# dmMaze/comic-text-detector

Measured on NVIDIA H100. Metric: pages/sec @1024x1024 synthetic, higher is better.
Workload: dtype fp16

## Files before the change

### comic-text-detector_b200/binding.py

```python
import ctypes as C
import os

import numpy as np

_HERE = os.path.dirname(os.path.abspath(__file__))
LIB_PATH = os.path.join(_HERE, "libctd_b200.so")
MAX_SRC = 3
ABI_VERSION = 2
PREC_FP16_TC, PREC_FP32_SIMT, PREC_FP16_SIMT, PREC_SPLIT_TC = 0, 1, 2, 3


class CtdOp(C.Structure):
    _fields_ = [("kind", C.c_int32), ("n_src", C.c_int32), ("src_buf", C.c_int32 * MAX_SRC),
                ("src_coff", C.c_int32 * MAX_SRC), ("src_c", C.c_int32 * MAX_SRC), ("dst_buf", C.c_int32),
                ("dst_coff", C.c_int32), ("cout", C.c_int32), ("cout_pad", C.c_int32), ("ksize", C.c_int32),
                ("stride", C.c_int32), ("act", C.c_int32), ("residual", C.c_int32), ("aux", C.c_int32),
                ("w16_off", C.c_int64), ("w32_off", C.c_int64), ("b_off", C.c_int64), ("p_off", C.c_int64)]


class CtdBufDesc(C.Structure):
    _fields_ = [("channels", C.c_int32), ("down", C.c_int32)]


class CtdConfig(C.Structure):
# ... 38 lines not shown
class CtdDevicePage(C.Structure):
    _fields_ = [("data", C.c_void_p), ("stride_h", C.c_int64), ("stride_w", C.c_int64), ("stride_c", C.c_int64),
                ("event", C.c_void_p)]


EXPORTS = ["ctd_create", "ctd_destroy", "ctd_last_error", "ctd_forward", "ctd_get_net_outputs", "ctd_get_mask_u8",
           "ctd_get_detections", "ctd_get_db_components", "ctd_last_forward_ms", "ctd_last_launch_count",
           "ctd_debug_read_buffer", "ctd_debug_write_buffer", "ctd_connected_components", "ctd_nms",
           "ctd_timer_start", "ctd_timer_stop", "ctd_profile_forward", "ctd_get_device_outputs",
           "ctd_get_text_lines", "ctd_seg_represent", "ctd_refine_mask", "ctd_submit", "ctd_collect",
           "ctd_results_bytes", "ctd_join", "ctd_forward_resized", "ctd_get_mask_u8_resized",
           "ctd_resize_linear_u8", "ctd_debug_run_ops", "ctd_get_nms_status", "ctd_group_output",
           "ctd_expand_textwindow", "ctd_detect_page", "ctd_results_layout", "ctd_submit_full", "ctd_device_arena",
           "ctd_region_plan", "ctd_transform_regions", "ctd_pages_plan", "ctd_submit_pages",
           "ctd_submit_pages_regions", "ctd_collect_regions", "ctd_submit_pages_device", "ctd_collect_device",
           "ctd_forward_tensor"]

_lib = None


class CtdError(RuntimeError):
    pass


def load_library():
    global _lib
    if _lib is not None:
        return _lib
    if not os.path.isfile(LIB_PATH):
        raise CtdError("libctd_b200.so is not built (%s); run `python -c 'import __graft_entry__ as g; g.build()'` "
                       "-- there is no CPU fallback" % LIB_PATH)
# ... 21 lines not shown
    lib.ctd_get_text_lines.argtypes = [vp, vp, vp, vp]
    lib.ctd_seg_represent.argtypes = [vp, vp, i32, i32, C.c_float, vp, vp, vp]
    lib.ctd_refine_mask.argtypes = [vp, vp, vp, i32, i32, vp, i32, i32, vp]
    lib.ctd_timer_start.argtypes = [vp]
    lib.ctd_timer_stop.argtypes = [vp, C.POINTER(C.c_float)]
    lib.ctd_profile_forward.argtypes = [vp, vp, i32, i32, i32, i32, vp, i32]
    lib.ctd_get_device_outputs.argtypes = [vp, C.POINTER(CtdDeviceOutputs)]
    lib.ctd_submit.argtypes = [vp, i32, vp, i32, i32, i32, vp]
    lib.ctd_collect.argtypes = [vp, i32]
    lib.ctd_results_bytes.argtypes = [vp, C.POINTER(C.c_size_t)]
    lib.ctd_join.argtypes = [vp, vp]
    lib.ctd_forward_resized.argtypes = [vp, vp, i32, i32, i32, i32, i32, i32]
    lib.ctd_get_mask_u8_resized.argtypes = [vp, i32, i32, i32, i32, vp]
    lib.ctd_resize_linear_u8.argtypes = [vp, vp, i32, i32, i32, vp, i32, i32]
    lib.ctd_debug_run_ops.argtypes = [vp, vp, i32, i32, i32, i32, i32]
    lib.ctd_get_nms_status.argtypes = [vp, vp, C.POINTER(i32)]
    lib.ctd_group_output.argtypes = [vp, vp, i32, vp, i32, i32, i32, vp, i32, vp, i32, vp, i32, vp, i32, C.POINTER(i32)]
    lib.ctd_expand_textwindow.argtypes = [i32, i32, vp, i32, vp]
    lib.ctd_detect_page.argtypes = [vp, vp, i32, i32, i32, i32, i32, i32, vp, vp, vp, i32, vp, i32, vp, i32, C.POINTER(i32)]
    lib.ctd_results_layout.argtypes = [vp, C.POINTER(CtdResultsLayout)]
    lib.ctd_submit_full.argtypes = [vp, i32, vp, i32, i32, i32, i32, i32, vp]
    lib.ctd_device_arena.argtypes = [vp, i32, C.POINTER(vp), C.POINTER(vp)]
    lib.ctd_region_plan.argtypes = [vp, i32, i32, i32, i32, vp, C.POINTER(C.c_size_t)]
    lib.ctd_transform_regions.argtypes = [vp, vp, i32, i32, i32, vp, i32, vp, C.c_size_t]
    lib.ctd_pages_plan.argtypes = [vp, i32, i32, i32, C.POINTER(C.c_size_t), C.POINTER(C.c_size_t)]
    lib.ctd_submit_pages.argtypes = [vp, i32, vp, i32, i32, i32, vp, i32, i32, vp]
    lib.ctd_submit_pages_regions.argtypes = [vp, i32, vp, i32, i32, i32, vp, i32, i32, i32, vp]
    lib.ctd_collect_regions.argtypes = [vp, i32, C.POINTER(vp), C.POINTER(i32), C.POINTER(vp), C.POINTER(vp),
                                        C.POINTER(C.c_size_t)]
    lib.ctd_submit_pages_device.argtypes = [vp, i32, vp, i32, i32, i32, vp, vp, i32, i32, i32, i32, vp]
# ... 212 lines not shown
        win = np.ascontiguousarray(np.asarray(windows, np.int32).reshape(-1, 4))
        out = np.empty(mask.shape, np.uint8)
        self._ck(self.lib.ctd_refine_mask(self.h, _ptr(img), _ptr(mask), mask.shape[0], mask.shape[1], _ptr(win), len(win),
                                          int(refine_mode), _ptr(out)))
        return out

    def last_forward_ms(self):
        ms = C.c_float()
        self._ck(self.lib.ctd_last_forward_ms(self.h, C.byref(ms)))
        return ms.value

    def last_launch_count(self):
        v = C.c_int32()
        self._ck(self.lib.ctd_last_launch_count(self.h, C.byref(v)))
        return v.value

    def debug_read(self, tensor):
        n, h, w = self.shape
        ch = self.program.bufs[tensor["buf"]][0]
        d = tensor["down"]
        out = np.empty((n, h // d, w // d, ch), np.float32)
        self._ck(self.lib.ctd_debug_read_buffer(self.h, tensor["buf"], _ptr(out), out.size))
        return out[..., tensor["coff"]:tensor["coff"] + tensor["c"]]

    def timer_start(self):
        self._ck(self.lib.ctd_timer_start(self.h))

    def timer_stop(self):
        ms = C.c_float()
        self._ck(self.lib.ctd_timer_stop(self.h, C.byref(ms)))
# ... 228 lines not shown
```

### comic-text-detector_b200/csrc/conv_tc.cu

```cuda
#include <cstdlib>
#include <cstring>
#include <cuda.h>
#include <cuda_fp16.h>
#include <cuda_runtime.h>

#include "kernels.h"
#include "ptx.cuh"

namespace ctd {

constexpr int kTileW = 16;
constexpr int kThreads = 384;

template <int BN, int TH>
struct TcCfg {
  static constexpr int kABytes = TH * kTileW * 128;
  static constexpr int kBBytes = BN * 128;
  static constexpr int kStages = TH == 8 ? (BN >= 128 ? 5 : (BN >= 64 ? 8 : 10))
                                         : (BN >= 128 ? 3 : (BN >= 64 ? 4 : (BN >= 32 ? 5 : 6)));
  static constexpr int kBoxN = BN < 64 ? BN : 64;
  static constexpr int kBoxBytes = 8 * TH * kBoxN * 2;
  static constexpr int kStgBytes = (BN / kBoxN) * kBoxBytes;
  static constexpr int kBiasFloats = 512;
  static constexpr size_t kSmem = 1024 + size_t(kStages) * (kABytes + kBBytes) + 2 * kStgBytes + 256 + kBiasFloats * 4;
// ... 82 lines not shown

template <int BN, int ACT>
__device__ __forceinline__ void epilogue_f32(const float (&acc)[BN / 2], const float* __restrict__ bias_s,
                                             float* const (&out)[2], const bool (&valid)[2], int ncols, int lane,
                                             bool residual) {
#pragma unroll
  for (int h = 0; h < 2; ++h) {
    if (!valid[h]) continue;
#pragma unroll
    for (int j = 0; j < BN / 8; ++j)
      epi_pair_f32<ACT>(acc[j * 4 + 2 * h], acc[j * 4 + 2 * h + 1], bias_s, j * 8 + (lane & 3) * 2, out[h], ncols,
                        residual);
  }
}

template <int BN, int TH>
__global__ void __launch_bounds__(kThreads, 1) conv_tc_kernel(const __grid_constant__ ConvTcParams p) {
  using Cfg = TcCfg<BN, TH>;
  constexpr int MT = TH / 8;
  extern __shared__ __align__(1024) uint8_t smem_tc[];
  const uint32_t raw_base = smem_u32(smem_tc);
  const uint32_t smem_base = (raw_base + 1023u) & ~1023u;
  uint8_t* const smem_gen = smem_tc + (smem_base - raw_base);
  const uint32_t a_base = smem_base;
  const uint32_t b_base = a_base + Cfg::kStages * Cfg::kABytes;
  const uint32_t stg_base = b_base + Cfg::kStages * Cfg::kBBytes;
  const uint32_t bar_base = stg_base + 2 * Cfg::kStgBytes;
  const uint32_t full_bar = bar_base, empty_bar = bar_base + 8 * Cfg::kStages, res_bar0 = bar_base + 16 * Cfg::kStages;
  float* bias_s = reinterpret_cast<float*>(smem_gen + (bar_base - smem_base) + 256);

  const int warp = threadIdx.x >> 5, lane = threadIdx.x & 31;
// ... 5 lines not shown
  int kblocks_per_tap = 0;
  for (int s = 0; s < g.n_src; ++s) kblocks_per_tap += p.src_kblocks[s];
  const int n_terms = p.split ? 3 : 1;
  const int its_per_tile = g.taps * kblocks_per_tap * n_terms;
  const int tiles_per_img = p.tiles_x * p.tiles_y;
  const int n_nblk = g.cout_pad / BN;
  const int spatial_tiles = g.n_img * tiles_per_img;
  const int total_tiles = spatial_tiles * n_nblk * g.n_phase;

  if (warp == 0 && lane == 0) {
    for (int s = 0; s < g.n_src; ++s)
      for (int q = 0; q < (g.in_stride == 2 ? 4 : 1); ++q) prefetch_tensormap(&p.a_map[s][q]);
    prefetch_tensormap(&p.b_map);
    if (p.dst != nullptr && !p.split)
      for (int ph = 0; ph < g.n_phase; ++ph) prefetch_tensormap(&p.d_map[ph]);
    for (int s = 0; s < Cfg::kStages; ++s) {
      mbar_init(full_bar + 8 * s, 1);
      mbar_init(empty_bar + 8 * s, 2);
    }
    mbar_init(res_bar0, 1);
    mbar_init(res_bar0 + 8, 1);
    fence_barrier_init();
  }
  for (int i = threadIdx.x; i < g.cout_pad && i < Cfg::kBiasFloats; i += kThreads) bias_s[i] = p.bias ? p.bias[i] : 0.f;
  __syncthreads();

  auto decode = [&](int t, int& phase, int& nblk, int& img, int& y0, int& x0) {
    nblk = t % n_nblk;
    const int r = t / n_nblk;
    const int sp = r % spatial_tiles;
    phase = r / spatial_tiles;
    img = sp / tiles_per_img;
    const int trem = sp - img * tiles_per_img;
    const int ty = trem / p.tiles_x;
    y0 = ty * TH;
    x0 = (trem - ty * p.tiles_x) * kTileW;
  };

  if (warp < 4) {
// ... 11 lines not shown
            for (int cb = 0; cb < p.src_kblocks[s]; ++cb) {
              for (int term = 0; term < n_terms; ++term, ++it) {
                const int stage = it % Cfg::kStages;
                const uint32_t par = ((it / Cfg::kStages) & 1) ^ 1;
                mbar_wait_relaxed(empty_bar + 8 * stage, par);
                mbar_arrive_expect_tx(full_bar + 8 * stage, stage_tx);
                tma_load_4d(a_base + stage * Cfg::kABytes, &p.a_map[s][q], full_bar + 8 * stage, cb * kb, x0 + dx,
                            y0 + dy, img + (term == 1 ? p.split_img_off : 0));
                tma_load_2d(b_base + stage * Cfg::kBBytes, &p.b_map, full_bar + 8 * stage, kglob + cb * kb,
                            phase * g.cout_pad + nblk * BN + (term == 2 ? p.split_row_off : 0));
              }
            }
            kglob += g.src_c[s];
          }
        }
      }
    }
    return;
  }

  if constexpr (TH == 16) setmaxnreg_inc<232>();
  const int wg = (warp >> 2) - 1;
  const int wrow = ((warp & 3) << 4) + (lane >> 2);
  const bool wg_leader = (threadIdx.x & 127) == 0;
  const uint64_t a_desc0 = make_kmajor_desc(a_base + uint32_t(wg * MT) * 64u * row_bytes, row_bytes);
  const uint64_t b_desc0 = make_kmajor_desc(b_base, row_bytes);
  const uint64_t a_mstep = (64u * row_bytes) >> 4;
  const int ksteps = kb / 16;
  int stage = 0;
  uint32_t full_par = 0;
// ... 11 lines not shown
    const int sy0 = y0 + wg * (TH / 2);
    if (res16 && wg_leader) {
      tma_store_wait_read();
      mbar_arrive_expect_tx(res_bar, Cfg::kStgBytes);
#pragma unroll
      for (int b = 0; b < BN / Cfg::kBoxN; ++b)
        tma_load_4d(stg + b * Cfg::kBoxBytes, &p.d_map[phase], res_bar, nblk * BN + b * Cfg::kBoxN, x0, sy0, img);
    }
    float acc[MT][R];
#pragma unroll
    for (int m = 0; m < MT; ++m)
#pragma unroll
      for (int i = 0; i < R; ++i) acc[m][i] = 0.f;

    bool split_done = false;
    if constexpr (BN <= 64 && TH == 8) {
      if (p.split) {
        float cross[R], tmp[R];
#pragma unroll
        for (int i = 0; i < R; ++i) cross[i] = 0.f;
        bool cross_started = false;
        for (int k_it = 0; k_it < its_per_tile; ++k_it) {
          mbar_wait(full_bar + 8 * stage, full_par);
          const uint64_t ad = a_desc0 + uint64_t(stage) * (Cfg::kABytes >> 4);
          const uint64_t bd = b_desc0 + uint64_t(stage) * (Cfg::kBBytes >> 4);
          if (k_it % 3 == 0) {
            for (int ks = 0; ks < ksteps; ++ks) {
              wgmma_fence();
              wgmma_bn<BN>(tmp, ad + 2 * ks, bd + 2 * ks, 0u);
              wgmma_commit();
              wgmma_wait<0>();
// ... 87 lines not shown
              if (((i >> 1) & 1) != h) continue;
              const int c = (i >> 2) * 8 + (lane & 3) * 2 + (i & 1), col = nblk * BN + c;
              if (col < p.dst_map_cols || col >= g.cout) continue;
              float f;
              switch (g.act) {
                case CTD_ACT_SILU: f = apply_act<CTD_ACT_SILU>(acc[m][i] + bias_t[c]); break;
                case CTD_ACT_LEAKY: f = apply_act<CTD_ACT_LEAKY>(acc[m][i] + bias_t[c]); break;
                case CTD_ACT_RELU: f = apply_act<CTD_ACT_RELU>(acc[m][i] + bias_t[c]); break;
                case CTD_ACT_SIGMOID: f = apply_act<CTD_ACT_SIGMOID>(acc[m][i] + bias_t[c]); break;
                default: f = acc[m][i] + bias_t[c]; break;
              }
              if (res16) f = __fadd_rn(f, __half2float(out[col]));
              out[col] = __float2half_rn(f);
            }
          }
      }
      continue;
    }
    const int ph_y = phase >> 1, ph_x = phase & 1;
    const int ncols = g.cout - nblk * BN;
#pragma unroll
    for (int m = 0; m < MT; ++m) {
      int gy[2], gx[2];
      bool valid[2];
      size_t pix[2];
#pragma unroll
      for (int h = 0; h < 2; ++h) {
        const int row = (wg * MT + m) * 64 + wrow + 8 * h;
        gy[h] = y0 + row / kTileW;
        gx[h] = x0 + row % kTileW;
// ... 43 lines not shown
  if (nhwc16 && wg_leader) tma_store_wait_all();
}


static const char* encode_map(PFN_encodeTiled enc, CUtensorMap* m, const void* base, int rank, const cuuint64_t* dims,
                              const cuuint64_t* strides_bytes, const cuuint32_t* box, int kb_elems) {
  cuuint32_t estr[5] = {1, 1, 1, 1, 1};
  const CUtensorMapSwizzle sw = kb_elems == 64 ? CU_TENSOR_MAP_SWIZZLE_128B
                                               : (kb_elems == 32 ? CU_TENSOR_MAP_SWIZZLE_64B : CU_TENSOR_MAP_SWIZZLE_32B);
  CUresult r = enc(m, CU_TENSOR_MAP_DATA_TYPE_FLOAT16, rank, const_cast<void*>(base), dims, strides_bytes, box, estr,
                   CU_TENSOR_MAP_INTERLEAVE_NONE, sw, CU_TENSOR_MAP_L2_PROMOTION_L2_256B,
                   CU_TENSOR_MAP_FLOAT_OOB_FILL_NONE);
  return r == CUDA_SUCCESS ? nullptr : "cuTensorMapEncodeTiled failed";
}

static const char* encode_dst_maps(PFN_encodeTiled enc, ConvTcParams& p, const __half* dst, int bn, int th) {
  const ConvGeom& g = p.g;
  const int boxn = bn < 64 ? bn : 64;
  p.dst_map_cols = g.cout & ~7;
  if (p.dst_map_cols == 0) return "conv_tc: fp16 destination needs at least 8 output channels";
  const cuuint64_t px = cuuint64_t(g.dst_cstride) * 2;
  for (int ph = 0; ph < g.n_phase; ++ph) {
    const int ph_y = ph >> 1, ph_x = ph & 1;
    const char* base = reinterpret_cast<const char*>(dst) + size_t(g.dst_coff) * 2 + (size_t(ph_y) * g.dst_w + ph_x) * px;
    cuuint64_t dims[4] = {cuuint64_t(p.dst_map_cols), cuuint64_t(g.gw), cuuint64_t(g.gh), cuuint64_t(g.n_img)};
    cuuint64_t str[3] = {px * g.out_mul, px * g.dst_w * g.out_mul, px * g.dst_w * g.dst_h};
    cuuint32_t box[4] = {cuuint32_t(boxn), kTileW, cuuint32_t(th / 2), 1};
    if (const char* e = encode_map(enc, &p.d_map[ph], base, 4, dims, str, box, boxn)) return e;
  }
  return nullptr;
}

static int g_num_sms = 132;

static int pick_block_n(int cout_pad) {
  if (cout_pad >= 128 && cout_pad % 128 == 0) return 128;
  if (cout_pad % 64 == 0) return 64;
  if (cout_pad % 32 == 0) return 32;
  return 16;
}

template <int TH>
static size_t smem_for(int bn) {
  switch (bn) {
    case 128: return TcCfg<128, TH>::kSmem;
    case 64: return TcCfg<64, TH>::kSmem;
    case 32: return TcCfg<32, TH>::kSmem;
    default: return TcCfg<16, TH>::kSmem;
  }
}

const char* conv_tc_plan(ConvTcPlan& plan, PFN_encodeTiled enc, const ConvGeom& g, const void* const src_ptr[],
                         const int src_coff[], const void* w16, const float* bias, __half* dst, int split) {
  ConvTcParams& p = plan.p;
  memset(&p, 0, sizeof(p));
  p.g = g;
  p.split = split ? 1 : 0;
  p.split_img_off = g.n_img;
  p.split_row_off = g.n_phase * g.cout_pad;
  const int n_planes = split ? 2 : 1;
  int kb = 64;
  for (int s = 0; s < g.n_src; ++s) {
    if (g.src_c[s] % 64 != 0 && kb > 32) kb = 32;
    if (g.src_c[s] % 32 != 0) kb = 16;
    if (g.src_c[s] % 16 != 0) return "conv_tc: source channels must be a multiple of 16";
    if (src_coff[s] % 8 != 0) return "conv_tc: source channel offset must be a multiple of 8";
  }
  if ((g.dst_coff % 8) != 0 || (g.dst_cstride % 8) != 0) return "conv_tc: destination slice must be 16-byte aligned";
  p.kb_elems = kb;
  for (int s = 0; s < g.n_src; ++s) p.src_kblocks[s] = g.src_c[s] / kb;
  p.tiles_x = (g.gw + kTileW - 1) / kTileW;
  int bn = pick_block_n(g.cout_pad);
  const int tiles8 = g.n_img * p.tiles_x * ((g.gh + 7) / 8) * g.n_phase;
  while (bn > 64 && tiles8 * (g.cout_pad / bn) <= g_num_sms / 2) bn /= 2;
  if (split && bn > 64) bn = 64;
  int th = 8;
  if (!split && dst != nullptr &&
      g.n_img * p.tiles_x * ((g.gh + 15) / 16) * g.n_phase * (g.cout_pad / bn) >= g_num_sms)
    th = 16;
// ... 22 lines not shown
  }
  for (int ph = 0; ph < g.n_phase; ++ph)
    for (int t = 0; t < g.taps; ++t) {
      if (g.in_stride == 2) {
        const int dy = g.tap_dy[ph][t], dx = g.tap_dx[ph][t];
        const int yp = dy != 0, xp = dx != 0;
        p.tap_map[ph][t] = int8_t(yp * 2 + xp);
        p.g.tap_dy[ph][t] = int8_t(dy < 0 ? -1 : 0);
        p.g.tap_dx[ph][t] = int8_t(dx < 0 ? -1 : 0);
      } else {
        p.tap_map[ph][t] = 0;
      }
    }
  plan.block_n = bn;
  plan.tile_h = th;
  if (dst != nullptr && !split)
    if (const char* e = encode_dst_maps(enc, p, dst, bn, th)) return e;
  if (split && ((g.dst_coff % 4) != 0 || (g.dst_cstride % 4) != 0 || (dst != nullptr && g.cout % 4 != 0)))
    return "conv_tc (split): fp32 destination slice must be 16-byte aligned";
  {
    cuuint64_t dims[2] = {cuuint64_t(g.k_total), cuuint64_t(g.n_phase) * cuuint64_t(g.cout_pad) * n_planes};
    cuuint64_t str[1] = {cuuint64_t(g.k_total) * 2};
    cuuint32_t box[2] = {cuuint32_t(kb), cuuint32_t(bn)};
    if (const char* e = encode_map(enc, &p.b_map, w16, 2, dims, str, box, kb)) return e;
  }
  {
    const int total_tiles = g.n_img * p.tiles_x * p.tiles_y * (g.cout_pad / bn) * g.n_phase;
    plan.grid = dim3(unsigned(total_tiles < g_num_sms ? total_tiles : g_num_sms), 1, 1);
  }
  if (g.cout_pad > 512) return "conv_tc: cout_pad > 512 not supported (bias staging)";
  plan.smem_bytes = th == 16 ? smem_for<16>(bn) : smem_for<8>(bn);
  return nullptr;
}

cudaError_t conv_tc_init() {
  cudaError_t e;
  int dev = 0;
  if (cudaGetDevice(&dev) == cudaSuccess) {
    int n = 0;
    if (cudaDeviceGetAttribute(&n, cudaDevAttrMultiProcessorCount, dev) == cudaSuccess && n > 0) g_num_sms = n;
  }
#define CTD_SET(BN, TH)                                                                                       \
  e = cudaFuncSetAttribute(conv_tc_kernel<BN, TH>, cudaFuncAttributeMaxDynamicSharedMemorySize,               \
                           int(TcCfg<BN, TH>::kSmem));                                                        \
  if (e != cudaSuccess) return e;
  CTD_SET(128, 8) CTD_SET(64, 8) CTD_SET(32, 8) CTD_SET(16, 8)
  CTD_SET(128, 16) CTD_SET(64, 16) CTD_SET(32, 16) CTD_SET(16, 16)
#undef CTD_SET
  return cudaSuccess;
}

template <int TH>
static void launch_th(const ConvTcPlan& plan, cudaStream_t s) {
  switch (plan.block_n) {
    case 128: conv_tc_kernel<128, TH><<<plan.grid, kThreads, plan.smem_bytes, s>>>(plan.p); break;
    case 64: conv_tc_kernel<64, TH><<<plan.grid, kThreads, plan.smem_bytes, s>>>(plan.p); break;
    case 32: conv_tc_kernel<32, TH><<<plan.grid, kThreads, plan.smem_bytes, s>>>(plan.p); break;
    default: conv_tc_kernel<16, TH><<<plan.grid, kThreads, plan.smem_bytes, s>>>(plan.p); break;
  }
}

cudaError_t conv_tc_launch(const ConvTcPlan& plan, cudaStream_t s) {
  if (plan.tile_h == 16) launch_th<16>(plan, s);
  else launch_th<8>(plan, s);
  return cudaGetLastError();
}

}
```

### comic-text-detector_b200/csrc/engine.cu

```cuda
#include <cuda.h>
#include <cuda_fp16.h>
#include <cuda_runtime.h>
#include <stdarg.h>
#include <stdio.h>
#include <string.h>

#include <algorithm>
#include <cstdlib>
#include <map>
#include <string>
#include <tuple>
#include <vector>

#include "engine.h"

using namespace ctd;

namespace {
thread_local std::string g_create_error;
}

int ctd_fail(ctd_handle* h, int code, const char* fmt, ...) {
  char buf[512];
  va_list ap;
// ... 263 lines not shown
  for (int l = 0; l < h->ops[i].aux; ++l) row0 += 3 * (ph / (8 << l)) * (pw / (8 << l));
  p.level_row0 = row0;
  p.nc = h->cfg.nc;
  p.det_stride = h->detect_prm[i][0];
  for (int k = 0; k < 6; ++k) p.anchor_wh[k] = h->detect_prm[i][1 + k];
}

static bool runs_on_tensor_cores(int precision, int kind) {
  switch (precision) {
    case CTD_PREC_SPLIT_TC: return is_gemm(kind);
    case CTD_PREC_FP16_TC: return is_gemm(kind) || kind == CTD_OP_STEM || kind == CTD_OP_SEG_TAIL;
    default: return false;
  }
}

static int build_plans(ctd_handle* h, int n, int ph, int pw, ShapePlan& sp) {
  sp.tc.resize(h->ops.size());
  sp.ends.resize(h->ops.size());
  const bool split = h->cfg.precision == CTD_PREC_SPLIT_TC;
  for (size_t i = 0; i < h->ops.size(); ++i) {
    const ctd_op& op = h->ops[i];
    if (!runs_on_tensor_cores(h->cfg.precision, op.kind)) continue;
    const float* bias = reinterpret_cast<const float*>(h->d_blob + op.b_off);
    const char* e = nullptr;
    if (op.kind == CTD_OP_STEM) {
      const bool f16 = sp.input == INPUT_F32;
      e = conv_ends_plan_stem(sp.ends[i], h->enc, f16 ? static_cast<const void*>(h->in_stage.p) : h->d_pages, f16, n,
                              ph, pw, h->d_blob + op.w16_off, bias, static_cast<__half*>(h->d_buf[op.dst_buf]),
                              h->bufs[op.dst_buf].channels, op.dst_coff, op.cout, op.act);
    } else if (op.kind == CTD_OP_SEG_TAIL) {
// ... 6 lines not shown
      ConvGeom g;
      if (int rc = op_geom(h, op, n, ph, pw, g)) return rc;
      const void* src[CTD_MAX_SRC];
      int coff[CTD_MAX_SRC];
      for (int s = 0; s < op.n_src; ++s) {
        src[s] = (split ? h->d_buf16 : h->d_buf)[op.src_buf[s]];
        coff[s] = op.src_coff[s];
      }
      const void* w = split ? h->d_wsplit + h->wsplit_off[i] : h->d_blob + op.w16_off;
      __half* dst = op.kind == CTD_OP_DETECT ? nullptr : static_cast<__half*>(h->d_buf[op.dst_buf]);
      e = conv_tc_plan(sp.tc[i], h->enc, g, src, coff, w, bias, dst, split);
      if (op.kind == CTD_OP_DETECT) set_detect(h, i, ph, pw, sp.tc[i].p);
    }
    if (e) return ctd_fail(h, CTD_E_INVALID, "op %zu: %s", i, e);
  }
  return CTD_OK;
}

template <typename T>
static int run_op_simt(ctd_handle* h, size_t i, int n, int ph, int pw) {
  const ctd_op& op = h->ops[i];
  ConvSimtParams p;
  memset(&p, 0, sizeof(p));
  if (int rc = op_geom(h, op, n, ph, pw, p.g)) return rc;
  for (int k = 0; k < op.n_src; ++k)
    p.src[k] = static_cast<char*>(h->d_buf[op.src_buf[k]]) + size_t(op.src_coff[k]) * sizeof(T);
  p.w = h->d_blob + (sizeof(T) == 4 ? op.w32_off : op.w16_off);
  p.bias = reinterpret_cast<const float*>(h->d_blob + op.b_off);
  if (op.kind == CTD_OP_DETECT) set_detect(h, i, ph, pw, p);
  else p.dst = h->d_buf[op.dst_buf];
  CK(conv_simt_launch<T>(p, h->stream));
// ... 63 lines not shown
  const ConvTcPlan& tc = sp.tc[i];
  int rc = CTD_OK;
  if (tc.block_n || sp.ends[i].kind != ctd::CTD_END_NONE) {
    const cudaError_t e = tc.block_n ? conv_tc_launch(tc, h->stream) : conv_ends_launch(sp.ends[i], h->stream);
    if (e != cudaSuccess) rc = ctd_fail(h, CTD_E_CUDA, "tensor-core op %zu: %s", i, cudaGetErrorString(e));
  } else if (is_gemm(op.kind)) {
    rc = h->elem == 4 ? run_op_simt<float>(h, i, n, ph, pw) : run_op_simt<__half>(h, i, n, ph, pw);
  } else {
    rc = h->elem == 4 ? run_op_thin<float>(h, op, n, ph, pw, sp.input) : run_op_thin<__half>(h, op, n, ph, pw, sp.input);
  }
  ++*cnt;
  if (rc || h->d_buf16.empty()) return rc;
  return split_written_slice(h, op, n, ph, pw, cnt);
}

static int launch_nms(ctd_handle* h, int n, int ph, int pw, cudaStream_t s, int* cnt) {
  CK(nms_launch(h->d_blks, n, rows_per_image(ph, pw), h->cfg.nc, h->cfg.conf_thresh, h->cfg.nms_thresh, h->nms, h->d_det,
                h->d_det_count, s));
  *cnt += kNmsLaunches;
  return CTD_OK;
}

static int launch_db_post(ctd_handle* h, int n, int ph, int pw, cudaStream_t s, int* cnt) {
  CK(ccl_launch(h->d_bitmap, n, ph, pw, h->d_labels, h->d_ccl_scratch, h->d_nlabels, s));
  CK(segrep_launch(h->d_bitmap, h->d_lines, size_t(2) * ph * pw, h->d_ccl_scratch, n, ph, pw, 1000, 1.5f,
                   h->d_segrep_scratch, h->d_line_boxes, h->d_line_scores, h->d_line_count, s));
  *cnt += kCclLaunches + kSegrepLaunches;
  return CTD_OK;
}

static int run_ops(ctd_handle* h, int n, int ph, int pw, const ShapePlan& sp, int* launches, bool record = false) {
  int cnt = 0;
  size_t evi = 0;
  if (h->overlap && !record && !h->cfg.debug_skip_postproc) {
    for (size_t i = 0; i < h->ops.size(); ++i)
      if (h->db_ancestor[i])
        if (int rc = run_one_op(h, i, n, ph, pw, sp, &cnt)) return rc;
    CK(cudaEventRecord(h->ev_fork, h->stream));
    CK(cudaStreamWaitEvent(h->side, h->ev_fork, 0));
    if (int rc = launch_db_post(h, n, ph, pw, h->side, &cnt)) return rc;
    CK(cudaEventRecord(h->ev_join, h->side));
    size_t last_detect = h->ops.size();
    for (size_t i = 0; i < h->ops.size(); ++i)
      if (!h->db_ancestor[i] && h->ops[i].kind == CTD_OP_DETECT) last_detect = i;
    bool nms_forked = false;
    for (size_t i = 0; i < h->ops.size(); ++i) {
      if (h->db_ancestor[i]) continue;
      if (int rc = run_one_op(h, i, n, ph, pw, sp, &cnt)) return rc;
      if (i == last_detect) {
        CK(cudaEventRecord(h->ev_fork2, h->stream));
        CK(cudaStreamWaitEvent(h->side2, h->ev_fork2, 0));
        if (int rc = launch_nms(h, n, ph, pw, h->side2, &cnt)) return rc;
        CK(cudaEventRecord(h->ev_join2, h->side2));
        nms_forked = true;
      }
    }
    if (!nms_forked) {
      if (int rc = launch_nms(h, n, ph, pw, h->stream, &cnt)) return rc;
    } else {
      CK(cudaStreamWaitEvent(h->stream, h->ev_join2, 0));
    }
    CK(cudaStreamWaitEvent(h->stream, h->ev_join, 0));
    *launches = cnt;
    return CTD_OK;
  }
  if (record) CK(cudaEventRecord(h->op_events[evi++], h->stream));
  for (size_t i = 0; i < h->ops.size(); ++i) {
    if (int rc = run_one_op(h, i, n, ph, pw, sp, &cnt)) return rc;
    if (record) CK(cudaEventRecord(h->op_events[evi++], h->stream));
  }
  *launches = cnt;
  if (h->cfg.debug_skip_postproc) return CTD_OK;
  if (int rc = launch_nms(h, n, ph, pw, h->stream, &cnt)) return rc;
  if (record) CK(cudaEventRecord(h->op_events[evi++], h->stream));
  if (int rc = launch_db_post(h, n, ph, pw, h->stream, &cnt)) return rc;
  if (record) CK(cudaEventRecord(h->op_events[evi++], h->stream));
  *launches = cnt;
  return CTD_OK;
}

static size_t stage_elem(const ctd_handle* h) { return h->cfg.precision == CTD_PREC_FP16_TC ? 2 : 4; }

static int find_plan(ctd_handle* h, int32_t n, int32_t ph, int32_t pw, ShapePlan** out, int input = INPUT_U8) {
// ... 451 lines not shown
  if (e == cudaSuccess) {
    if (h->elem == 4) from_f32_kernel<float><<<unsigned((elems + 255) / 256), 256, 0, h->stream>>>(tmp, static_cast<float*>(h->d_buf[buf]), elems);
    else from_f32_kernel<__half><<<unsigned((elems + 255) / 256), 256, 0, h->stream>>>(tmp, static_cast<__half*>(h->d_buf[buf]), elems);
    if (h->cfg.precision == CTD_PREC_SPLIT_TC) {
      const size_t npix = elems / b.channels;
      __half* hi = static_cast<__half*>(h->d_buf16[buf]);
      e = split_planes_launch(static_cast<const float*>(h->d_buf[buf]), hi, hi + elems, npix, b.channels, b.channels, h->stream);
    }
    if (e == cudaSuccess) e = cudaStreamSynchronize(h->stream);
  }
  cudaFree(tmp);
  CK(e);
  return CTD_OK;
}

extern "C" int ctd_debug_run_ops(ctd_handle* h, const uint8_t* pages, int32_t n, int32_t ph, int32_t pw, int32_t first_op,
                                 int32_t last_op) {
  if (!h) return CTD_E_INVALID;
  if (first_op < 0 || last_op >= int(h->ops.size()) || first_op > last_op) return ctd_fail(h, CTD_E_INVALID, "bad op range");
  ShapePlan* sp = nullptr;
  if (int rc = find_plan(h, n, ph, pw, &sp)) return rc;
  if (pages) CK(cudaMemcpyAsync(h->d_pages, pages, size_t(n) * ph * pw * 3, cudaMemcpyHostToDevice, h->stream));
  int cnt = 0;
  for (int i = first_op; i <= last_op; ++i)
    if (int rc = run_one_op(h, size_t(i), n, ph, pw, *sp, &cnt)) return rc;
  CK(cudaStreamSynchronize(h->stream));
  h->n = n; h->ph = ph; h->pw = pw;
  h->have_forward = true;
  h->last_launches = cnt;
  return CTD_OK;
// ... 53 lines not shown
```

### comic-text-detector_b200/csrc/engine.h

```cpp
#pragma once
#include <cuda.h>
#include <cuda_runtime.h>
#include <stdint.h>

#include <math.h>

#include <algorithm>
#include <array>
#include <condition_variable>
#include <deque>
#include <map>
#include <mutex>
#include <optional>
#include <string>
#include <thread>
#include <tuple>
#include <vector>

#include "kernels.h"

using ctd::ConvTcPlan;
using ctd::ConvEndsPlan;
using ctd::NmsWorkspace;
using ctd::PFN_encodeTiled;
// ... 114 lines not shown
struct RegionJob {
  std::vector<ctd::RegionDev> regs;
  std::vector<ctd::RegionTile> tiles;
  size_t out_bytes = 0;
  int add(const ctd_region* plan, int n, long long page_off, int ih, int iw, long long out_base);
  size_t table_bytes() const;
  void write_tables(char* dst) const;
};

enum { INPUT_U8 = 0, INPUT_F32 = 1 };

struct ShapePlan {
  int input = INPUT_U8;
  std::vector<ConvTcPlan> tc;
  std::vector<ConvEndsPlan> ends;
  cudaGraphExec_t graph = nullptr;
  int launches = 0;
};
struct ctd_handle {
  ctd_config cfg{};
  std::vector<ctd_op> ops;
  std::vector<ctd_bufdesc> bufs;
  std::vector<std::array<float, 7>> detect_prm;
  std::string err;
  cudaStream_t stream = nullptr;
  cudaEvent_t ev0 = nullptr, ev1 = nullptr, tev0 = nullptr, tev1 = nullptr;
  std::vector<cudaEvent_t> op_events;
  PFN_encodeTiled enc = nullptr;
  char* d_blob = nullptr;
  size_t blob_bytes = 0;
// ... 67 lines not shown
```

### comic-text-detector_b200/csrc/kernels.h

```cpp
#pragma once
#include <cuda.h>
#include <cuda_fp16.h>
#include <cuda_runtime.h>
#include <stdint.h>

#include "../../include/ctd_b200.h"

namespace ctd {

constexpr int kMaxTaps = 9;

constexpr float kSplitLoScale = 2048.0f;
constexpr float kSplitLoUnscale = 1.0f / 2048.0f;
constexpr int kMaxPhases = 4;

struct ConvGeom {
  int n_img;
  int gh, gw;
  int dst_h, dst_w;
  int out_mul;
  int n_phase;
  int taps;
  int cin_total;
  int k_total;
// ... 20 lines not shown
  int src_kblocks[CTD_MAX_SRC];
  int tiles_x, tiles_y;
  int8_t tap_map[kMaxPhases][kMaxTaps];
  __half* dst;
  int dst_map_cols;
  const float* bias;
  float* blks;
  int blks_rows_per_img;
  int level_row0;
  float det_stride;
  float anchor_wh[6];
  int nc;
  int split;
  int split_img_off;
  int split_row_off;
};
static_assert(sizeof(ConvTcParams) <= 4096, "ConvTcParams: kernel parameters are limited to 4 KB");

struct ConvTcPlan {
  ConvTcParams p;
  int block_n;
  int tile_h;
  dim3 grid;
  size_t smem_bytes;
};

typedef CUresult (*PFN_encodeTiled)(CUtensorMap*, CUtensorMapDataType, cuuint32_t, void*, const cuuint64_t*,
                                    const cuuint64_t*, const cuuint32_t*, const cuuint32_t*, CUtensorMapInterleave,
                                    CUtensorMapSwizzle, CUtensorMapL2promotion, CUtensorMapFloatOOBfill);

const char* conv_tc_plan(ConvTcPlan& plan, PFN_encodeTiled enc, const ConvGeom& g, const void* const src_ptr[],
                         const int src_coff[], const void* w16, const float* bias, __half* dst, int split = 0);
cudaError_t conv_tc_launch(const ConvTcPlan& plan, cudaStream_t s);
cudaError_t conv_tc_init();

enum { CTD_END_NONE = 0, CTD_END_STEM = 1, CTD_END_SEG = 2, CTD_END_STEM_F16 = 3 };
struct alignas(64) ConvEndsParams {
  CUtensorMap a_map;
  CUtensorMap b_map;
  CUtensorMap d_map;
  int n_img, gh, gw;
  int tiles_x, tiles_y;
  const float* bias;
  float* mask_f32;
  uint8_t* mask_u8;
};
struct ConvEndsPlan {
// ... 127 lines not shown
```

### include/ctd_b200.h

```cpp
#ifndef CTD_B200_H_
#define CTD_B200_H_

#include <stddef.h>
#include <stdint.h>

#ifdef __cplusplus
extern "C" {
#endif

#define CTD_ABI_VERSION 2
#if defined(__GNUC__)
#define CTD_API __attribute__((visibility("default")))
#else
#define CTD_API
#endif

#define CTD_OK 0
#define CTD_E_INVALID (-1)
#define CTD_E_CUDA (-2)
#define CTD_E_NO_DEVICE (-3)
#define CTD_E_SHAPE (-4)
#define CTD_E_CAPACITY (-5)


// ... 92 lines not shown

CTD_API int ctd_submit(ctd_handle* h, int32_t slot, const uint8_t* pages_host, int32_t n, int32_t ph, int32_t pw,
                       void* results_host);
CTD_API int ctd_collect(ctd_handle* h, int32_t slot);
CTD_API int ctd_results_bytes(ctd_handle* h, size_t* bytes);

CTD_API int ctd_join(ctd_handle* h, ctd_handle* other);

CTD_API int ctd_last_forward_ms(ctd_handle* h, float* ms);
CTD_API int ctd_last_launch_count(ctd_handle* h, int32_t* launches);
CTD_API int ctd_debug_read_buffer(ctd_handle* h, int32_t buf, float* out, size_t out_elems);
CTD_API int ctd_debug_write_buffer(ctd_handle* h, int32_t buf, const float* in, int32_t n, int32_t ph, int32_t pw);

CTD_API int ctd_debug_run_ops(ctd_handle* h, const uint8_t* pages, int32_t n, int32_t ph, int32_t pw, int32_t first_op,
                              int32_t last_op);

CTD_API int ctd_timer_start(ctd_handle* h);
CTD_API int ctd_timer_stop(ctd_handle* h, float* ms);
CTD_API int ctd_profile_forward(ctd_handle* h, const uint8_t* pages, int32_t n, int32_t ph, int32_t pw,
                                int32_t pages_on_device, float* op_ms, int32_t cap);
typedef struct ctd_device_outputs {
  void* stream;
  void* mask_u8;
  void* det;
  void* det_count;
  void* bitmap;
  void* labels;
  void* n_labels;
  void* line_boxes;
  void* line_scores;
// ... 116 lines not shown
```

Before: 1119.

## Fuse 1x1 follower convolutions into producer tensor-core conv epilogue

When a tensor-core conv is immediately followed by a 1x1 conv that reads a slice of its output, the producer kernel now runs the follower GEMM from its staged fp16 output tile in shared memory and stores the follower result via TMA. This removes the follower's separate launch and its re-read of the intermediate activation from global memory. It adds new kernel template instantiations, a larger parameter block and extra serial wgmma work in the producer's epilogue, which can lengthen the producer kernel and raise register pressure.

```diff
diff --git a/comic-text-detector_b200/binding.py b/comic-text-detector_b200/binding.py
--- a/comic-text-detector_b200/binding.py
+++ b/comic-text-detector_b200/binding.py
@@ -76,7 +76,7 @@
            "ctd_expand_textwindow", "ctd_detect_page", "ctd_results_layout", "ctd_submit_full", "ctd_device_arena",
            "ctd_region_plan", "ctd_transform_regions", "ctd_pages_plan", "ctd_submit_pages",
            "ctd_submit_pages_regions", "ctd_collect_regions", "ctd_submit_pages_device", "ctd_collect_device",
-           "ctd_forward_tensor"]
+           "ctd_forward_tensor", "ctd_fused_ops"]
 
 _lib = None
 
@@ -128,6 +128,7 @@
     lib.ctd_get_mask_u8_resized.argtypes = [vp, i32, i32, i32, i32, vp]
     lib.ctd_resize_linear_u8.argtypes = [vp, vp, i32, i32, i32, vp, i32, i32]
     lib.ctd_debug_run_ops.argtypes = [vp, vp, i32, i32, i32, i32, i32]
+    lib.ctd_fused_ops.argtypes = [vp, i32, i32, i32, vp, i32, C.POINTER(i32)]
     lib.ctd_get_nms_status.argtypes = [vp, vp, C.POINTER(i32)]
     lib.ctd_group_output.argtypes = [vp, vp, i32, vp, i32, i32, i32, vp, i32, vp, i32, vp, i32, vp, i32, C.POINTER(i32)]
     lib.ctd_expand_textwindow.argtypes = [i32, i32, vp, i32, vp]
@@ -370,6 +371,13 @@
         v = C.c_int32()
         self._ck(self.lib.ctd_last_launch_count(self.h, C.byref(v)))
         return v.value
+
+    def fused_pairs(self, n, h, w):
+        cap = len(self.program.ops)
+        prod = np.zeros((max(cap, 1),), np.int32)
+        k = C.c_int32()
+        self._ck(self.lib.ctd_fused_ops(self.h, n, h, w, _ptr(prod), cap, C.byref(k)))
+        return [(int(p), int(p) + 1) for p in prod[:k.value]]
 
     def debug_read(self, tensor):
         n, h, w = self.shape
diff --git a/comic-text-detector_b200/csrc/conv_tc.cu b/comic-text-detector_b200/csrc/conv_tc.cu
--- a/comic-text-detector_b200/csrc/conv_tc.cu
+++ b/comic-text-detector_b200/csrc/conv_tc.cu
@@ -120,7 +120,7 @@
   }
 }
 
-template <int BN, int TH>
+template <int BN, int TH, int NF>
 __global__ void __launch_bounds__(kThreads, 1) conv_tc_kernel(const __grid_constant__ ConvTcParams p) {
   using Cfg = TcCfg<BN, TH>;
   constexpr int MT = TH / 8;
@@ -156,6 +156,10 @@
     prefetch_tensormap(&p.b_map);
     if (p.dst != nullptr && !p.split)
       for (int ph = 0; ph < g.n_phase; ++ph) prefetch_tensormap(&p.d_map[ph]);
+    if constexpr (NF > 0) {
+      prefetch_tensormap(&p.f_b_map);
+      for (int ph = 0; ph < g.n_phase; ++ph) prefetch_tensormap(&p.f_d_map[ph]);
+    }
     for (int s = 0; s < Cfg::kStages; ++s) {
       mbar_init(full_bar + 8 * s, 1);
       mbar_init(empty_bar + 8 * s, 2);
@@ -165,6 +169,8 @@
     fence_barrier_init();
   }
   for (int i = threadIdx.x; i < g.cout_pad && i < Cfg::kBiasFloats; i += kThreads) bias_s[i] = p.bias ? p.bias[i] : 0.f;
+  if constexpr (NF > 0)
+    for (int i = threadIdx.x; i < p.f_cout_pad; i += kThreads) bias_s[g.cout_pad + i] = p.f_bias[i];
   __syncthreads();
 
   auto decode = [&](int t, int& phase, int& nblk, int& img, int& y0, int& x0) {
@@ -206,6 +212,18 @@
             kglob += g.src_c[s];
           }
         }
+        if constexpr (NF > 0) {
+          if (nblk == p.f_nblk) {
+            const uint32_t f_tx = uint32_t(NF) * uint32_t(p.f_kb_elems) * 2u;
+            for (int fk = 0; fk < p.f_kblocks; ++fk, ++it) {
+              const int stage = it % Cfg::kStages;
+              const uint32_t par = ((it / Cfg::kStages) & 1) ^ 1;
+              mbar_wait_relaxed(empty_bar + 8 * stage, par);
+              mbar_arrive_expect_tx(full_bar + 8 * stage, f_tx);
+              tma_load_2d(b_base + stage * Cfg::kBBytes, &p.f_b_map, full_bar + 8 * stage, fk * p.f_kb_elems, 0);
+            }
+          }
+        }
       }
     }
     return;
@@ -247,7 +265,7 @@
       for (int i = 0; i < R; ++i) acc[m][i] = 0.f;
 
     bool split_done = false;
-    if constexpr (BN <= 64 && TH == 8) {
+    if constexpr (BN <= 64 && TH == 8 && NF == 0) {
       if (p.split) {
         float cross[R], tmp[R];
 #pragma unroll
@@ -365,6 +383,57 @@
               out[col] = __float2half_rn(f);
             }
           }
+      }
+      if constexpr (NF > 0) {
+        if (nblk == p.f_nblk) {
+          using FCfg = TcCfg<NF, TH>;
+          constexpr uint32_t kStgRow = Cfg::kBoxN * 2;
+          const int fks = p.f_kb_elems / 16;
+          const uint64_t fb_desc0 = make_kmajor_desc(b_base, uint32_t(p.f_kb_elems) * 2u);
+          using FAcc = float[NF / 2];
+          FAcc* facc = reinterpret_cast<FAcc*>(&acc[0][0]);
+          static_assert(sizeof(acc[0]) == sizeof(FAcc) * (BN / NF), "follower accumulators");
+          for (int fk = 0; fk < p.f_kblocks; ++fk) {
+            mbar_wait(full_bar + 8 * stage, full_par);
+            const uint64_t bd = fb_desc0 + uint64_t(stage) * (Cfg::kBBytes >> 4);
+            wgmma_fence();
+            for (int ks = 0; ks < fks; ++ks) {
+              const int kc = p.f_koff + fk * p.f_kb_elems + ks * 16;
+              const uint64_t ad = make_kmajor_desc(stg + uint32_t(kc / Cfg::kBoxN) * Cfg::kBoxBytes, kStgRow) +
+                                  uint64_t(kc % Cfg::kBoxN) / 8;
+#pragma unroll
+              for (int m = 0; m < MT; ++m)
+                wgmma_bn<NF>(facc[m * (BN / NF)], ad + m * ((64u * kStgRow) >> 4), bd + 2 * ks, (fk > 0 || ks > 0) ? 1u : 0u);
+            }
+            wgmma_commit();
+            wgmma_wait<0>();
+            if (wg_leader) mbar_arrive(empty_bar + 8 * stage);
+            if (++stage == Cfg::kStages) { stage = 0; full_par ^= 1u; }
+          }
+#pragma unroll
+          for (int m = 0; m < MT; ++m) wgmma_fence_regs(facc[m * (BN / NF)]);
+          if (wg_leader) tma_store_wait_read();
+          named_barrier_sync(epi_bar, 128);
+          const float* f_bias = bias_s + g.cout_pad;
+#define CTD_FEPI(ACT) \
+  _Pragma("unroll") for (int m = 0; m < MT; ++m) stage_f16<NF, TH, ACT, false>(facc[m * (BN / NF)], f_bias, stg, m, warp & 3, lane);
+          switch (p.f_act) {
+            case CTD_ACT_SILU: CTD_FEPI(CTD_ACT_SILU) break;
+            case CTD_ACT_LEAKY: CTD_FEPI(CTD_ACT_LEAKY) break;
+            case CTD_ACT_RELU: CTD_FEPI(CTD_ACT_RELU) break;
+            case CTD_ACT_SIGMOID: CTD_FEPI(CTD_ACT_SIGMOID) break;
+            default: CTD_FEPI(CTD_ACT_NONE) break;
+          }
+#undef CTD_FEPI
+          fence_proxy_async();
+          named_barrier_sync(epi_bar, 128);
+          if (wg_leader) {
+#pragma unroll
+            for (int b = 0; b < NF / FCfg::kBoxN; ++b)
+              tma_store_4d(&p.f_d_map[phase], stg + b * FCfg::kBoxBytes, b * FCfg::kBoxN, x0, sy0, img);
+            tma_store_commit();
+          }
+        }
       }
       continue;
     }
@@ -438,19 +507,19 @@
   return r == CUDA_SUCCESS ? nullptr : "cuTensorMapEncodeTiled failed";
 }
 
-static const char* encode_dst_maps(PFN_encodeTiled enc, ConvTcParams& p, const __half* dst, int bn, int th) {
-  const ConvGeom& g = p.g;
+static const char* encode_dst_maps(PFN_encodeTiled enc, CUtensorMap (&maps)[kMaxPhases], const ConvGeom& g,
+                                   const __half* dst, int bn, int th) {
   const int boxn = bn < 64 ? bn : 64;
-  p.dst_map_cols = g.cout & ~7;
-  if (p.dst_map_cols == 0) return "conv_tc: fp16 destination needs at least 8 output channels";
+  const int cols = g.cout & ~7;
+  if (cols == 0) return "conv_tc: fp16 destination needs at least 8 output channels";
   const cuuint64_t px = cuuint64_t(g.dst_cstride) * 2;
   for (int ph = 0; ph < g.n_phase; ++ph) {
     const int ph_y = ph >> 1, ph_x = ph & 1;
     const char* base = reinterpret_cast<const char*>(dst) + size_t(g.dst_coff) * 2 + (size_t(ph_y) * g.dst_w + ph_x) * px;
-    cuuint64_t dims[4] = {cuuint64_t(p.dst_map_cols), cuuint64_t(g.gw), cuuint64_t(g.gh), cuuint64_t(g.n_img)};
+    cuuint64_t dims[4] = {cuuint64_t(cols), cuuint64_t(g.gw), cuuint64_t(g.gh), cuuint64_t(g.n_img)};
     cuuint64_t str[3] = {px * g.out_mul, px * g.dst_w * g.out_mul, px * g.dst_w * g.dst_h};
     cuuint32_t box[4] = {cuuint32_t(boxn), kTileW, cuuint32_t(th / 2), 1};
-    if (const char* e = encode_map(enc, &p.d_map[ph], base, 4, dims, str, box, boxn)) return e;
+    if (const char* e = encode_map(enc, &maps[ph], base, 4, dims, str, box, boxn)) return e;
   }
   return nullptr;
 }
@@ -472,6 +541,15 @@
     case 32: return TcCfg<32, TH>::kSmem;
     default: return TcCfg<16, TH>::kSmem;
   }
+}
+
+static int k_block(const ConvGeom& g) {
+  int kb = 64;
+  for (int s = 0; s < g.n_src; ++s) {
+    if (g.src_c[s] % 64 != 0 && kb > 32) kb = 32;
+    if (g.src_c[s] % 32 != 0) kb = 16;
+  }
+  return kb;
 }
 
 const char* conv_tc_plan(ConvTcPlan& plan, PFN_encodeTiled enc, const ConvGeom& g, const void* const src_ptr[],
@@ -483,10 +561,8 @@
   p.split_img_off = g.n_img;
   p.split_row_off = g.n_phase * g.cout_pad;
   const int n_planes = split ? 2 : 1;
-  int kb = 64;
+  const int kb = k_block(g);
   for (int s = 0; s < g.n_src; ++s) {
-    if (g.src_c[s] % 64 != 0 && kb > 32) kb = 32;
-    if (g.src_c[s] % 32 != 0) kb = 16;
     if (g.src_c[s] % 16 != 0) return "conv_tc: source channels must be a multiple of 16";
     if (src_coff[s] % 8 != 0) return "conv_tc: source channel offset must be a multiple of 8";
   }
@@ -539,8 +615,10 @@
     }
   plan.block_n = bn;
   plan.tile_h = th;
-  if (dst != nullptr && !split)
-    if (const char* e = encode_dst_maps(enc, p, dst, bn, th)) return e;
+  if (dst != nullptr && !split) {
+    p.dst_map_cols = g.cout & ~7;
+    if (const char* e = encode_dst_maps(enc, p.d_map, g, dst, bn, th)) return e;
+  }
   if (split && ((g.dst_coff % 4) != 0 || (g.dst_cstride % 4) != 0 || (dst != nullptr && g.cout % 4 != 0)))
     return "conv_tc (split): fp32 destination slice must be 16-byte aligned";
   {
@@ -558,6 +636,43 @@
   return nullptr;
 }
 
+bool conv_tc_add_follower(ConvTcPlan& plan, PFN_encodeTiled enc, const ConvGeom& fg, int f_src_off, const void* w16,
+                          const float* bias, __half* dst, const char** err) {
+  *err = nullptr;
+  ConvTcParams& p = plan.p;
+  const ConvGeom& g = p.g;
+  const int bn = plan.block_n, cin = fg.cin_total;
+  if (p.split || p.dst == nullptr || (bn != 64 && bn != 128) || plan.follow_n != 0) return false;
+  if (fg.taps != 1 || fg.n_phase != 1 || fg.in_stride != 1 || fg.n_src != 1 || fg.residual != 0) return false;
+  if (f_src_off < 0 || cin <= 0 || f_src_off + cin > p.dst_map_cols) return false;
+  const int nblk = f_src_off / bn, koff = f_src_off - nblk * bn;
+  if (koff + cin > bn || koff % 16 != 0) return false;
+  if (g.cout_pad != bn) return false;
+  if ((fg.cout_pad != 32 && fg.cout_pad != 64 && fg.cout_pad != 128) || fg.cout_pad > bn) return false;
+  if (fg.cout % 8 != 0 || g.cout_pad + fg.cout_pad > TcCfg<128, 8>::kBiasFloats) return false;
+  const int kb = k_block(fg);
+  {
+    cuuint64_t dims[2] = {cuuint64_t(cin), cuuint64_t(fg.cout_pad)};
+    cuuint64_t str[1] = {cuuint64_t(cin) * 2};
+    cuuint32_t box[2] = {cuuint32_t(kb), cuuint32_t(fg.cout_pad)};
+    if ((*err = encode_map(enc, &p.f_b_map, w16, 2, dims, str, box, kb))) return false;
+  }
+  ConvGeom dg = g;
+  dg.dst_cstride = fg.dst_cstride;
+  dg.dst_coff = fg.dst_coff;
+  dg.cout = fg.cout;
+  if ((*err = encode_dst_maps(enc, p.f_d_map, dg, dst, fg.cout_pad, plan.tile_h))) return false;
+  p.f_bias = bias;
+  p.f_nblk = nblk;
+  p.f_koff = koff;
+  p.f_kb_elems = kb;
+  p.f_kblocks = cin / kb;
+  p.f_cout_pad = fg.cout_pad;
+  p.f_act = fg.act;
+  plan.follow_n = fg.cout_pad;
+  return true;
+}
+
 cudaError_t conv_tc_init() {
   cudaError_t e;
   int dev = 0;
@@ -565,23 +680,43 @@
     int n = 0;
     if (cudaDeviceGetAttribute(&n, cudaDevAttrMultiProcessorCount, dev) == cudaSuccess && n > 0) g_num_sms = n;
   }
-#define CTD_SET(BN, TH)                                                                                       \
-  e = cudaFuncSetAttribute(conv_tc_kernel<BN, TH>, cudaFuncAttributeMaxDynamicSharedMemorySize,               \
+#define CTD_SET(BN, TH, NF)                                                                                   \
+  e = cudaFuncSetAttribute(conv_tc_kernel<BN, TH, NF>, cudaFuncAttributeMaxDynamicSharedMemorySize,           \
                            int(TcCfg<BN, TH>::kSmem));                                                        \
   if (e != cudaSuccess) return e;
-  CTD_SET(128, 8) CTD_SET(64, 8) CTD_SET(32, 8) CTD_SET(16, 8)
-  CTD_SET(128, 16) CTD_SET(64, 16) CTD_SET(32, 16) CTD_SET(16, 16)
+  CTD_SET(128, 8, 0) CTD_SET(64, 8, 0) CTD_SET(32, 8, 0) CTD_SET(16, 8, 0)
+  CTD_SET(128, 16, 0) CTD_SET(64, 16, 0) CTD_SET(32, 16, 0) CTD_SET(16, 16, 0)
+  CTD_SET(128, 8, 128) CTD_SET(128, 8, 64) CTD_SET(128, 8, 32) CTD_SET(64, 8, 64) CTD_SET(64, 8, 32)
+  CTD_SET(128, 16, 128) CTD_SET(128, 16, 64) CTD_SET(128, 16, 32) CTD_SET(64, 16, 64) CTD_SET(64, 16, 32)
 #undef CTD_SET
   return cudaSuccess;
+}
+
+template <int BN, int TH>
+static void launch_bn(const ConvTcPlan& plan, cudaStream_t s) {
+  if constexpr (BN >= 64) {
+    switch (plan.follow_n) {
+      case 32: conv_tc_kernel<BN, TH, 32><<<plan.grid, kThreads, plan.smem_bytes, s>>>(plan.p); return;
+      case 64: conv_tc_kernel<BN, TH, 64><<<plan.grid, kThreads, plan.smem_bytes, s>>>(plan.p); return;
+      case 128:
+        if constexpr (BN >= 128) {
+          conv_tc_kernel<BN, TH, 128><<<plan.grid, kThreads, plan.smem_bytes, s>>>(plan.p);
+          return;
+        }
+        break;
+      default: break;
+    }
+  }
+  conv_tc_kernel<BN, TH, 0><<<plan.grid, kThreads, plan.smem_bytes, s>>>(plan.p);
 }
 
 template <int TH>
 static void launch_th(const ConvTcPlan& plan, cudaStream_t s) {
   switch (plan.block_n) {
-    case 128: conv_tc_kernel<128, TH><<<plan.grid, kThreads, plan.smem_bytes, s>>>(plan.p); break;
-    case 64: conv_tc_kernel<64, TH><<<plan.grid, kThreads, plan.smem_bytes, s>>>(plan.p); break;
-    case 32: conv_tc_kernel<32, TH><<<plan.grid, kThreads, plan.smem_bytes, s>>>(plan.p); break;
-    default: conv_tc_kernel<16, TH><<<plan.grid, kThreads, plan.smem_bytes, s>>>(plan.p); break;
+    case 128: launch_bn<128, TH>(plan, s); break;
+    case 64: launch_bn<64, TH>(plan, s); break;
+    case 32: launch_bn<32, TH>(plan, s); break;
+    default: launch_bn<16, TH>(plan, s); break;
   }
 }
 
diff --git a/comic-text-detector_b200/csrc/engine.cu b/comic-text-detector_b200/csrc/engine.cu
--- a/comic-text-detector_b200/csrc/engine.cu
+++ b/comic-text-detector_b200/csrc/engine.cu
@@ -301,6 +301,45 @@
   }
 }
 
+static bool slices_overlap(int b, int c0, int c, int e, int d0, int d) {
+  return b >= 0 && b == e && c0 < d0 + d && d0 < c0 + c;
+}
+
+static int build_followers(ctd_handle* h, int n, int ph, int pw, ShapePlan& sp) {
+  const size_t n_ops = h->ops.size();
+  sp.fused.assign(n_ops, ConvTcPlan());
+  sp.n_fused = 0;
+  if (h->cfg.precision != CTD_PREC_FP16_TC) return CTD_OK;
+  std::vector<ConvTcPlan> cand(n_ops);
+  for (size_t i = 0; i + 1 < n_ops; ++i) {
+    const ctd_op& P = h->ops[i];
+    const ctd_op& F = h->ops[i + 1];
+    if (!sp.tc[i].block_n || !sp.tc[i + 1].block_n || (P.kind != CTD_OP_CONV && P.kind != CTD_OP_DECONV4)) continue;
+    if (F.kind != CTD_OP_CONV || F.ksize != 1 || F.stride != 1 || F.n_src != 1 || F.residual) continue;
+    if (h->db_ancestor[i] != h->db_ancestor[i + 1] || F.src_buf[0] != P.dst_buf) continue;
+    bool clash = slices_overlap(F.dst_buf, F.dst_coff, F.cout, P.dst_buf, P.dst_coff, P.cout);
+    for (int s = 0; s < P.n_src; ++s)
+      clash = clash || slices_overlap(F.dst_buf, F.dst_coff, F.cout, P.src_buf[s], P.src_coff[s], P.src_c[s]);
+    if (clash) continue;
+    ConvGeom fg;
+    if (int rc = op_geom(h, F, n, ph, pw, fg)) return rc;
+    ConvTcPlan plan = sp.tc[i];
+    const char* e = nullptr;
+    if (conv_tc_add_follower(plan, h->enc, fg, F.src_coff[0] - P.dst_coff, h->d_blob + F.w16_off,
+                             reinterpret_cast<const float*>(h->d_blob + F.b_off), static_cast<__half*>(h->d_buf[F.dst_buf]),
+                             &e))
+      cand[i] = plan;
+    else if (e)
+      return ctd_fail(h, CTD_E_INVALID, "op %zu with follower %zu: %s", i, i + 1, e);
+  }
+  for (size_t i = 0; i + 1 < n_ops; ++i)
+    if (cand[i].follow_n && !cand[i + 1].follow_n) {
+      sp.fused[i] = cand[i];
+      ++sp.n_fused;
+    }
+  return CTD_OK;
+}
+
 static int build_plans(ctd_handle* h, int n, int ph, int pw, ShapePlan& sp) {
   sp.tc.resize(h->ops.size());
   sp.ends.resize(h->ops.size());
@@ -337,7 +376,7 @@
     }
     if (e) return ctd_fail(h, CTD_E_INVALID, "op %zu: %s", i, e);
   }
-  return CTD_OK;
+  return build_followers(h, n, ph, pw, sp);
 }
 
 template <typename T>
@@ -431,6 +470,15 @@
   return split_written_slice(h, op, n, ph, pw, cnt);
 }
 
+static int run_planned_op(ctd_handle* h, size_t i, int n, int ph, int pw, const ShapePlan& sp, int* cnt) {
+  if (i > 0 && sp.fused[i - 1].follow_n) return CTD_OK;
+  if (!sp.fused[i].follow_n) return run_one_op(h, i, n, ph, pw, sp, cnt);
+  ++*cnt;
+  const cudaError_t e = conv_tc_launch(sp.fused[i], h->stream);
+  if (e != cudaSuccess) return ctd_fail(h, CTD_E_CUDA, "tensor-core op %zu with follower %zu: %s", i, i + 1, cudaGetErrorString(e));
+  return CTD_OK;
+}
+
 static int launch_nms(ctd_handle* h, int n, int ph, int pw, cudaStream_t s, int* cnt) {
   CK(nms_launch(h->d_blks, n, rows_per_image(ph, pw), h->cfg.nc, h->cfg.conf_thresh, h->cfg.nms_thresh, h->nms, h->d_det,
                 h->d_det_count, s));
@@ -452,7 +500,7 @@
   if (h->overlap && !record && !h->cfg.debug_skip_postproc) {
     for (size_t i = 0; i < h->ops.size(); ++i)
       if (h->db_ancestor[i])
-        if (int rc = run_one_op(h, i, n, ph, pw, sp, &cnt)) return rc;
+        if (int rc = run_planned_op(h, i, n, ph, pw, sp, &cnt)) return rc;
     CK(cudaEventRecord(h->ev_fork, h->stream));
     CK(cudaStreamWaitEvent(h->side, h->ev_fork, 0));
     if (int rc = launch_db_post(h, n, ph, pw, h->side, &cnt)) return rc;
@@ -463,7 +511,7 @@
     bool nms_forked = false;
     for (size_t i = 0; i < h->ops.size(); ++i) {
       if (h->db_ancestor[i]) continue;
-      if (int rc = run_one_op(h, i, n, ph, pw, sp, &cnt)) return rc;
+      if (int rc = run_planned_op(h, i, n, ph, pw, sp, &cnt)) return rc;
       if (i == last_detect) {
         CK(cudaEventRecord(h->ev_fork2, h->stream));
         CK(cudaStreamWaitEvent(h->side2, h->ev_fork2, 0));
@@ -483,7 +531,7 @@
   }
   if (record) CK(cudaEventRecord(h->op_events[evi++], h->stream));
   for (size_t i = 0; i < h->ops.size(); ++i) {
-    if (int rc = run_one_op(h, i, n, ph, pw, sp, &cnt)) return rc;
+    if (int rc = run_planned_op(h, i, n, ph, pw, sp, &cnt)) return rc;
     if (record) CK(cudaEventRecord(h->op_events[evi++], h->stream));
   }
   *launches = cnt;
@@ -965,6 +1013,21 @@
   return CTD_OK;
 }
 
+extern "C" int ctd_fused_ops(ctd_handle* h, int32_t n, int32_t ph, int32_t pw, int32_t* producers, int32_t cap,
+                             int32_t* count) {
+  if (!h || !count || (cap > 0 && !producers)) return CTD_E_INVALID;
+  ShapePlan* sp = nullptr;
+  if (int rc = find_plan(h, n, ph, pw, &sp)) return rc;
+  int k = 0;
+  for (size_t i = 0; i < sp->fused.size(); ++i)
+    if (sp->fused[i].follow_n) {
+      if (k < cap) producers[k] = int32_t(i);
+      ++k;
+    }
+  *count = k;
+  return CTD_OK;
+}
+
 extern "C" int ctd_debug_run_ops(ctd_handle* h, const uint8_t* pages, int32_t n, int32_t ph, int32_t pw, int32_t first_op,
                                  int32_t last_op) {
   if (!h) return CTD_E_INVALID;
diff --git a/comic-text-detector_b200/csrc/engine.h b/comic-text-detector_b200/csrc/engine.h
--- a/comic-text-detector_b200/csrc/engine.h
+++ b/comic-text-detector_b200/csrc/engine.h
@@ -152,6 +152,8 @@
   int input = INPUT_U8;
   std::vector<ConvTcPlan> tc;
   std::vector<ConvEndsPlan> ends;
+  std::vector<ConvTcPlan> fused;
+  int n_fused = 0;
   cudaGraphExec_t graph = nullptr;
   int launches = 0;
 };
diff --git a/comic-text-detector_b200/csrc/kernels.h b/comic-text-detector_b200/csrc/kernels.h
--- a/comic-text-detector_b200/csrc/kernels.h
+++ b/comic-text-detector_b200/csrc/kernels.h
@@ -58,6 +58,13 @@
   int split;
   int split_img_off;
   int split_row_off;
+  CUtensorMap f_b_map;
+  CUtensorMap f_d_map[kMaxPhases];
+  const float* f_bias;
+  int f_nblk;
+  int f_koff;
+  int f_kb_elems, f_kblocks;
+  int f_cout_pad, f_act;
 };
 static_assert(sizeof(ConvTcParams) <= 4096, "ConvTcParams: kernel parameters are limited to 4 KB");
 
@@ -65,6 +72,7 @@
   ConvTcParams p;
   int block_n;
   int tile_h;
+  int follow_n = 0;
   dim3 grid;
   size_t smem_bytes;
 };
@@ -75,6 +83,8 @@
 
 const char* conv_tc_plan(ConvTcPlan& plan, PFN_encodeTiled enc, const ConvGeom& g, const void* const src_ptr[],
                          const int src_coff[], const void* w16, const float* bias, __half* dst, int split = 0);
+bool conv_tc_add_follower(ConvTcPlan& plan, PFN_encodeTiled enc, const ConvGeom& fg, int f_src_off, const void* w16,
+                          const float* bias, __half* dst, const char** err);
 cudaError_t conv_tc_launch(const ConvTcPlan& plan, cudaStream_t s);
 cudaError_t conv_tc_init();
 
diff --git a/include/ctd_b200.h b/include/ctd_b200.h
--- a/include/ctd_b200.h
+++ b/include/ctd_b200.h
@@ -130,6 +130,9 @@
 
 CTD_API int ctd_debug_run_ops(ctd_handle* h, const uint8_t* pages, int32_t n, int32_t ph, int32_t pw, int32_t first_op,
                               int32_t last_op);
+
+CTD_API int ctd_fused_ops(ctd_handle* h, int32_t n, int32_t ph, int32_t pw, int32_t* producers, int32_t cap,
+                          int32_t* count);
 
 CTD_API int ctd_timer_start(ctd_handle* h);
 CTD_API int ctd_timer_stop(ctd_handle* h, float* ms);
```

Result: no change. 1136, median of 6 (+1.6%).
